# polli-labs/linnaeus

Measured on AMD Instinct MI355X. Metric: images/sec (train fwd+bwd) mFormerV1_sm 3x224x224, higher is better.
Workload: dtype bf16; 1 GPU; mFormerV1_sm train step (forward + 4-task CE loss + backward + AdamW (one HIP launch)), bf16 operands / fp32 accumulate+residual, batch 256/GPU, 3x224x224 synthetic, DropPath 0.2, gradient checkpointing off; per_gpu_batch=256, global_batch=256, parallelism=dp1, grad_mode=direct

## Files before the change

linnaeus_amd/csrc/convmlp.hip:

```cpp
#include <stdlib.h>

#include "common.hpp"
#include "../../include/lnx.h"

namespace {

struct CmP {
    const unsigned char* ln;
    const unsigned char* w1;
    const unsigned char* w2;
    const unsigned char* w2t;
    const unsigned char* w1t;
    const unsigned char* zin;
    const float* b1;
    const float* b2;
    const float* gamma;
    const float* rowscale;
    const float* x;
    const float* g;
    float* out;
    unsigned char* z;
    unsigned char* act;
    unsigned char* dh;
    unsigned char* dz;
    unsigned char* dln;
    float* dgamma;
    int M, C, rps;
    const unsigned char* y;
    const float* lnw;
    const float* lnb;
    float eps;
    unsigned char* ln_out;
    float* mean;
    float* rstd;
    float* part;
    int64_t part_floats;
    int ln_defer;
    int tile_slot;
    int dz_plain;
    float* dlnw;
    float* dlnb;
};

__device__ __forceinline__ void mfma16(f32x4_t& acc, const uint4& a, const uint4& b) {
    acc = __builtin_amdgcn_mfma_f32_16x16x32_bf16(__builtin_bit_cast(bf16x8_t, a), __builtin_bit_cast(bf16x8_t, b), acc, 0, 0, 0);
}

__device__ __forceinline__ int key4(int a) { return (4 - (a & 3)) & 3; }

#define CM_DS_READ128(dst, addr, OFF) asm volatile("ds_read_b128 %0, %1 offset:" #OFF : "=v"(dst) : "v"(addr) : "memory")

template <int NK> struct Geo {
    static constexpr int C = 32 * NK;
    static constexpr int PART = NK * 4096;
    static constexpr int CT = C / 16;
};

template <int NK, int NW>
__device__ __forceinline__ void dma_nmajor(unsigned char* lds_part, const unsigned char* W, int n0, int wave, int lane) {
    constexpr int C = Geo<NK>::C;
    constexpr int NINS = 4 * NK;
    static_assert(NINS % NW == 0, "DMA pieces must divide evenly over the waves");
#pragma unroll
    for (int t = 0; t < NINS / NW; ++t) {
        const int i = wave + NW * t;
        const int ks = i >> 2, rb = i & 3;
        const int row = 16 * rb + (lane >> 2), u = lane & 3;
        const unsigned char* src = W + ((int64_t)(n0 + row) * C + ks * 32 + ((u ^ key4(row >> 3)) << 3)) * 2;
        __builtin_amdgcn_global_load_lds((const __attribute__((address_space(1))) void*)src,
                                         (__attribute__((address_space(3))) void*)(lds_part + i * 1024), 16, 0, 0);
    }
}

template <int NK, int NW>
__device__ __forceinline__ void dma_cmajor(unsigned char* lds_part, const unsigned char* W, int n0, int wave, int lane) {
    constexpr int C = Geo<NK>::C;
    constexpr int RB = C / 16;
    constexpr int NINS = 2 * RB;
#pragma unroll
    for (int t = 0; t < NINS / NW; ++t) {
        const int i = wave + NW * t;
        const int ks2 = i / RB, rb = i % RB;
        const int row = 16 * rb + (lane >> 2), u = lane & 3;
// ... 72 lines not shown
#pragma unroll
    for (int ks2 = 0; ks2 < 2; ++ks2) {
#pragma unroll
        for (int c0 = 0; c0 < CT; c0 += GB) {
            uint4 wf[GB];
#pragma unroll
            for (int b = 0; b < GB; ++b) {
                const uint32_t a = base + (uint32_t)(ks2 * C * 64 + (c0 + b) * 1024);
                CM_DS_READ128(wf[b], a, 0);
            }
            asm volatile("s_waitcnt lgkmcnt(0)" ::: "memory");
            __builtin_amdgcn_sched_barrier(0);
#pragma unroll
            for (int b = 0; b < GB; ++b)
#pragma unroll
                for (int mt = 0; mt < MT; ++mt) mfma16(o[c0 + b][mt], wf[b], pf[mt][ks2]);
        }
    }
}

template <int NK, int MT>
__device__ __forceinline__ void prod_nmajor_pipe(f32x4_t (&h)[4][MT], uint32_t part_addr, int s, int g, const uint4 (&xf)[MT][NK]) {
    const uint32_t unit = (uint32_t)((g ^ key4(s >> 2)) << 4);
    const uint32_t base = part_addr + (uint32_t)((8 * (s >> 2) + (s & 3)) * 64) + unit;
#pragma unroll
    for (int nt = 0; nt < 4; ++nt)
#pragma unroll
        for (int mt = 0; mt < MT; ++mt) h[nt][mt] = f32x4_t{0.f, 0.f, 0.f, 0.f};
    uint4 wf[2][4];
    CM_DS_READ128(wf[0][0], base, 0);
    CM_DS_READ128(wf[0][1], base, 256);
    CM_DS_READ128(wf[0][2], base, 2048);
    CM_DS_READ128(wf[0][3], base, 2304);
#pragma unroll
    for (int ks = 0; ks < NK; ++ks) {
        if (ks + 1 < NK) {
            const uint32_t a = base + (ks + 1) * 4096;
            CM_DS_READ128(wf[(ks + 1) & 1][0], a, 0);
            CM_DS_READ128(wf[(ks + 1) & 1][1], a, 256);
            CM_DS_READ128(wf[(ks + 1) & 1][2], a, 2048);
            CM_DS_READ128(wf[(ks + 1) & 1][3], a, 2304);
            asm volatile("s_waitcnt lgkmcnt(4)" ::: "memory");
        } else {
            asm volatile("s_waitcnt lgkmcnt(0)" ::: "memory");
        }
        __builtin_amdgcn_sched_barrier(0);
#pragma unroll
        for (int nt = 0; nt < 4; ++nt)
#pragma unroll
            for (int mt = 0; mt < MT; ++mt) mfma16(h[nt][mt], wf[ks & 1][nt], xf[mt][ks]);
    }
}

template <int NK, int MT>
__device__ __forceinline__ void prod_cmajor_pipe(f32x4_t (&o)[Geo<NK>::CT][MT], uint32_t part_addr, int s, int g, const uint4 (&pf)[MT][2]) {
    constexpr int C = Geo<NK>::C;
    constexpr int CT = Geo<NK>::CT;
    const uint32_t base = part_addr + (uint32_t)(s * 64) + (uint32_t)((g ^ key4(s >> 2)) << 4);
    constexpr int GB = 4;
    constexpr int NB = 2 * CT / GB;
    static_assert(CT % GB == 0, "channel tiles must split into batches of 4");
    uint4 wf[2][GB];
#pragma unroll
    for (int b = 0; b < GB; ++b) CM_DS_READ128(wf[0][b], base + (uint32_t)(b * 1024), 0);
#pragma unroll
    for (int bt = 0; bt < NB; ++bt) {
        const int ks2 = (bt * GB) / CT, c0 = (bt * GB) % CT;
        if (bt + 1 < NB) {
            const int ks2n = ((bt + 1) * GB) / CT, c0n = ((bt + 1) * GB) % CT;
#pragma unroll
            for (int b = 0; b < GB; ++b) CM_DS_READ128(wf[(bt + 1) & 1][b], base + (uint32_t)(ks2n * C * 64 + (c0n + b) * 1024), 0);
            asm volatile("s_waitcnt lgkmcnt(4)" ::: "memory");
        } else {
            asm volatile("s_waitcnt lgkmcnt(0)" ::: "memory");
        }
        __builtin_amdgcn_sched_barrier(0);
#pragma unroll
        for (int b = 0; b < GB; ++b)
#pragma unroll
            for (int mt = 0; mt < MT; ++mt) mfma16(o[c0 + b][mt], wf[bt & 1][b], pf[mt][ks2]);
    }
}

__device__ __forceinline__ uint4 pack8(const f32x4_t& lo, const f32x4_t& hi) {
    Vec16<bf16_t> v;
#pragma unroll
    for (int j = 0; j < 4; ++j) {
        v.set(j, lo[j]);
        v.set(4 + j, hi[j]);
    }
    return v.raw;
}

__device__ __forceinline__ float g_sum(float v) {
    v += __shfl_xor(v, 16, 64);
    v += __shfl_xor(v, 32, 64);
    return v;
}
template <int CTRL> __device__ __forceinline__ float dpp_get(float v) {
    return __builtin_bit_cast(float, __builtin_amdgcn_update_dpp(0, __builtin_bit_cast(int, v), CTRL, 0xf, 0xf, false));
}
__device__ __forceinline__ float row16_sum(float v) {
    v += dpp_get<0xB1>(v);
    v += dpp_get<0x4E>(v);
    v += dpp_get<0x141>(v);
    v += dpp_get<0x140>(v);
    return v;
}
template <int NK>
__device__ __forceinline__ void ln_row_frags(uint4 (&xf)[NK], const float* w, const float* b, int g, float eps, float& mu, float& rs) {
    constexpr float invC = 1.0f / (float)Geo<NK>::C;
    float v[NK][8];
    float sum = 0.f;
#pragma unroll
    for (int ks = 0; ks < NK; ++ks) {
        Vec16<bf16_t> t;
        t.raw = xf[ks];
#pragma unroll
        for (int j = 0; j < 8; ++j) v[ks][j] = t.get(j);
        sum += ((v[ks][0] + v[ks][1]) + (v[ks][2] + v[ks][3])) + ((v[ks][4] + v[ks][5]) + (v[ks][6] + v[ks][7]));
    }
    mu = g_sum(sum) * invC;
    float sq = 0.f;
#pragma unroll
    for (int ks = 0; ks < NK; ++ks)
#pragma unroll
        for (int j = 0; j < 8; ++j) {
            v[ks][j] -= mu;
            sq = fmaf(v[ks][j], v[ks][j], sq);
        }
    rs = 1.0f / sqrtf(fmaf(g_sum(sq), invC, eps));
#pragma unroll
    for (int ks = 0; ks < NK; ++ks) {
        const int c = ks * 32 + 8 * g;
        const float4 w0 = *reinterpret_cast<const float4*>(w + c), w1 = *reinterpret_cast<const float4*>(w + c + 4);
        const float4 b0 = *reinterpret_cast<const float4*>(b + c), b1 = *reinterpret_cast<const float4*>(b + c + 4);
        const float wv[8] = {w0.x, w0.y, w0.z, w0.w, w1.x, w1.y, w1.z, w1.w};
        const float bv[8] = {b0.x, b0.y, b0.z, b0.w, b1.x, b1.y, b1.z, b1.w};
        Vec16<bf16_t> o;
#pragma unroll
        for (int j = 0; j < 8; ++j) o.set(j, fmaf(v[ks][j] * rs, wv[j], bv[j]));
        xf[ks] = o.raw;
    }
}
template <int NK>
struct LnRow {
    uint2 yr[Geo<NK>::CT];
    float mu, rs;
};
template <int NK>
__device__ __forceinline__ void ln_bwd_fetch(LnRow<NK>& r, const CmP& p, int m, int g) {
    constexpr int C = Geo<NK>::C;
    const int mc = m < p.M ? m : p.M - 1;
#pragma unroll
    for (int ct = 0; ct < Geo<NK>::CT; ++ct) r.yr[ct] = *reinterpret_cast<const uint2*>(p.y + ((int64_t)mc * C + ct * 16 + 4 * g) * 2);
    r.mu = p.mean[mc];
    r.rs = p.rstd[mc];
}
template <int NK, int MT, int MTI>
__device__ __forceinline__ void ln_bwd_rows(const CmP& p, const f32x4_t (&dl)[Geo<NK>::CT][MT], const LnRow<NK>& row, int m, int s, int g, const float* lnws,
                                            float* dls) {
    constexpr int C = Geo<NK>::C;
    constexpr int CT = Geo<NK>::CT;
    constexpr float invC = 1.0f / (float)C;
    const bool mv = m < p.M;
    const int mc = mv ? m : p.M - 1;
    const uint2 (&yr)[CT] = row.yr;
    const float mu = row.mu, rs = row.rs;
    float xh[CT][4], gv[CT][4];
    float s1 = 0.f, s2 = 0.f;
#pragma unroll
    for (int ct = 0; ct < CT; ++ct) {
        const int c = ct * 16 + 4 * g;
        const float4 w4 = *reinterpret_cast<const float4*>(lnws + c);
        const float wv[4] = {w4.x, w4.y, w4.z, w4.w};
        const bf16_t* yh = reinterpret_cast<const bf16_t*>(&yr[ct]);
#pragma unroll
        for (int r = 0; r < 4; ++r) {
            const float d = (float)(bf16_t)dl[ct][MTI][r];
            const float x = ((float)yh[r] - mu) * rs;
            xh[ct][r] = x;
            gv[ct][r] = d * wv[r];
            s1 += gv[ct][r];
            s2 = fmaf(gv[ct][r], x, s2);
            const float dm = mv ? d : 0.f;
            const float a = row16_sum(dm * x), b = row16_sum(dm);
            if (s == 0) {
                atomicAdd(&dls[c + r], a);
                atomicAdd(&dls[C + c + r], b);
            }
        }
    }
    const float m1 = g_sum(s1) * invC, m2 = g_sum(s2) * invC;
#pragma unroll
    for (int ct = 0; ct < CT; ++ct) {
        uint2 v;
        bf16_t* vh = reinterpret_cast<bf16_t*>(&v);
#pragma unroll
        for (int r = 0; r < 4; ++r) vh[r] = (bf16_t)(rs * (gv[ct][r] - m1 - xh[ct][r] * m2));
        *reinterpret_cast<uint2*>(p.dln + ((int64_t)mc * C + ct * 16 + 4 * g) * 2) = v;
    }
}

#ifdef CM_STAMP
__device__ unsigned long long g_cm_stamp[8];
#define CM_T(i) do { __builtin_amdgcn_sched_barrier(0); unsigned long long t_; asm volatile("s_memtime %0\n\ts_waitcnt lgkmcnt(0)" : "=s"(t_) :: "memory"); \
                     __builtin_amdgcn_sched_barrier(0); tsum[i] += t_ - tlast; tlast = t_; } while (0)
#else
#define CM_T(i) do { } while (0)
#endif

template <int NK, int MT, int NW, bool LNF>
__global__ __launch_bounds__(64 * NW) void convmlp_fwd_kernel(const CmP p) {
#ifdef CM_STAMP
    unsigned long long tsum[8] = {0, 0, 0, 0, 0, 0, 0, 0}, tlast;
    asm volatile("s_memtime %0\n\ts_waitcnt lgkmcnt(0)" : "=s"(tlast)::"memory");
#endif
    constexpr int C = Geo<NK>::C;
    constexpr int CT = Geo<NK>::CT;
    constexpr int PART = Geo<NK>::PART;
    constexpr int STAGE = 2 * PART;
    constexpr int NCH = 4 * C / 64;
    constexpr int NLD = 8 * NK / NW;
    extern __shared__ __attribute__((aligned(16))) unsigned char smem[];
    float* b1s = reinterpret_cast<float*>(smem + 3 * STAGE);

    const int lane = threadIdx.x & 63;
    const int wave = __builtin_amdgcn_readfirstlane(threadIdx.x >> 6);
    const int s = lane & 15, g = lane >> 4;
    const int m_base = blockIdx.x * (16 * NW * MT) + wave * (16 * MT);
    const uint32_t lds0 = (uint32_t)(uintptr_t)(__attribute__((address_space(3))) unsigned char*)smem;

    for (int i = threadIdx.x; i < 4 * C; i += 64 * NW) b1s[i] = p.b1[i];

    uint4 xf[MT][NK];
#pragma unroll
    for (int mt = 0; mt < MT; ++mt) {
        int m = m_base + mt * 16 + s;
        if (m >= p.M) m = p.M - 1;
#pragma unroll
        for (int ks = 0; ks < NK; ++ks) xf[mt][ks] = ld16((LNF ? p.y : p.ln) + ((int64_t)m * C + ks * 32 + 8 * g) * 2);
    }
    if constexpr (LNF) {
#pragma unroll
        for (int mt = 0; mt < MT; ++mt) {
            float mu, rs;
            ln_row_frags<NK>(xf[mt], p.lnw, p.lnb, g, p.eps, mu, rs);
            const int m = m_base + mt * 16 + s;
            if (m < p.M) {
                if (p.ln_out) {
#pragma unroll
                    for (int ks = 0; ks < NK; ++ks) st16(p.ln_out + ((int64_t)m * C + ks * 32 + 8 * g) * 2, xf[mt][ks]);
                }
                if (p.mean && g == 0) {
                    p.mean[m] = mu;
                    p.rstd[m] = rs;
                }
            }
        }
    }
    f32x4_t o[CT][MT];
#pragma unroll
    for (int ct = 0; ct < CT; ++ct)
#pragma unroll
        for (int mt = 0; mt < MT; ++mt) o[ct][mt] = f32x4_t{0.f, 0.f, 0.f, 0.f};

    __syncthreads();
    dma_nmajor<NK, NW>(smem, p.w1, 0, wave, lane);
    dma_cmajor<NK, NW>(smem + PART, p.w2, 0, wave, lane);
    dma_nmajor<NK, NW>(smem + STAGE, p.w1, 64, wave, lane);
    dma_cmajor<NK, NW>(smem + STAGE + PART, p.w2, 64, wave, lane);
    CM_T(0);
    for (int j = 0; j < NCH; ++j) {
        const int stg = j % 3;
        if (j + 1 < NCH) asm volatile("s_waitcnt vmcnt(%0)" ::"n"(NLD) : "memory");
        else asm volatile("s_waitcnt vmcnt(0)" ::: "memory");
        CM_T(1);
        __builtin_amdgcn_s_barrier();
        CM_T(2);
        if (j + 2 < NCH) {
            unsigned char* nx = smem + ((j + 2) % 3) * STAGE;
            dma_nmajor<NK, NW>(nx, p.w1, 64 * (j + 2), wave, lane);
            dma_cmajor<NK, NW>(nx + PART, p.w2, 64 * (j + 2), wave, lane);
        }
        const uint32_t st = lds0 + stg * STAGE;
        f32x4_t h[4][MT];
        CM_T(3);
        prod_nmajor_pipe<NK, MT>(h, st, s, g, xf);
        CM_T(4);
        uint4 pf[MT][2];
        {
            f32x4_t bv[4];
            const uint32_t ba = lds0 + 3 * STAGE + (uint32_t)((64 * j + 8 * g) * 4);
            CM_DS_READ128(bv[0], ba, 0);
            CM_DS_READ128(bv[1], ba, 16);
            CM_DS_READ128(bv[2], ba, 128);
            CM_DS_READ128(bv[3], ba, 144);
            asm volatile("s_waitcnt lgkmcnt(0)" ::: "memory");
            __builtin_amdgcn_sched_barrier(0);
#pragma unroll
            for (int mt = 0; mt < MT; ++mt)
#pragma unroll
                for (int n2 = 0; n2 < 4; n2 += 2) {
                    f32x4_t hv[2] = {h[n2][mt], h[n2 + 1][mt]};
                    gelu4_bias_n<2>(hv, &bv[n2]);
                    h[n2][mt] = hv[0];
                    h[n2 + 1][mt] = hv[1];
                }
#pragma unroll
            for (int mt = 0; mt < MT; ++mt) {
                pf[mt][0] = pack8(h[0][mt], h[1][mt]);
                pf[mt][1] = pack8(h[2][mt], h[3][mt]);
            }
        }
        CM_T(5);
        prod_cmajor_pipe<NK, MT>(o, st + PART, s, g, pf);
        CM_T(6);
    }
#pragma unroll
    for (int mt = 0; mt < MT; ++mt) {
        const int m = m_base + mt * 16 + s;
        if (m >= p.M) continue;
        const float rs = p.rowscale ? p.rowscale[m / p.rps] : 1.0f;
        float4 xrv[CT], b2v[CT], gmv[CT];
#pragma unroll
        for (int ct = 0; ct < CT; ++ct) {
            const int c = ct * 16 + 4 * g;
            xrv[ct] = *reinterpret_cast<const float4*>(p.x + (int64_t)m * C + c);
            b2v[ct] = *reinterpret_cast<const float4*>(p.b2 + c);
            gmv[ct] = *reinterpret_cast<const float4*>(p.gamma + c);
        }
#pragma unroll
        for (int ct = 0; ct < CT; ++ct) {
            const int c = ct * 16 + 4 * g;
            const float4 b2 = b2v[ct], gm = gmv[ct], xr = xrv[ct];
            const float z0 = o[ct][mt][0] + b2.x, z1 = o[ct][mt][1] + b2.y, z2 = o[ct][mt][2] + b2.z, z3 = o[ct][mt][3] + b2.w;
            if (p.z) {
                uint2 zz;
                bf16_t* zh = reinterpret_cast<bf16_t*>(&zz);
                zh[0] = (bf16_t)z0; zh[1] = (bf16_t)z1; zh[2] = (bf16_t)z2; zh[3] = (bf16_t)z3;
                *reinterpret_cast<uint2*>(p.z + ((int64_t)m * C + c) * 2) = zz;
            }
            *reinterpret_cast<float4*>(p.out + (int64_t)m * C + c) =
                make_float4(xr.x + rs * gm.x * z0, xr.y + rs * gm.y * z1, xr.z + rs * gm.z * z2, xr.w + rs * gm.w * z3);
        }
    }
    CM_T(7);
#ifdef CM_STAMP
    if (blockIdx.x == gridDim.x / 2 && threadIdx.x == 0)
        for (int i = 0; i < 8; ++i) g_cm_stamp[i] = tsum[i];
#endif
}
#ifdef CM_STAMP
extern "C" int lnx_dbg_convmlp_stamps(unsigned long long* out8) { return (int)hipMemcpyFromSymbol(out8, HIP_SYMBOL(g_cm_stamp), 64); }
#endif

template <int NK, int MT, int NW, bool ST, bool LNB, bool DG>
__global__ __launch_bounds__(64 * NW) void convmlp_bwd_kernel(const CmP p) {
    constexpr int C = Geo<NK>::C;
    constexpr int CT = Geo<NK>::CT;
    constexpr int PART = Geo<NK>::PART;
    constexpr int STAGE = 3 * PART;
    constexpr int NCH = 4 * C / 64;
    constexpr int NLD = 12 * NK / NW;
    extern __shared__ __attribute__((aligned(16))) unsigned char smem[];
    float* b1s = reinterpret_cast<float*>(smem + 2 * STAGE);
    float* dgs = b1s + 4 * C;
    float* lws = dgs + C;
    float* dls = lws + C;

    const int lane = threadIdx.x & 63;
    const int wave = __builtin_amdgcn_readfirstlane(threadIdx.x >> 6);
    const int s = lane & 15, g = lane >> 4;
    const int m_base = blockIdx.x * (16 * NW * MT) + wave * (16 * MT);
    const uint32_t lds0 = (uint32_t)(uintptr_t)(__attribute__((address_space(3))) unsigned char*)smem;

    for (int i = threadIdx.x; i < 4 * C; i += 64 * NW) b1s[i] = p.b1[i];
    for (int i = threadIdx.x; i < C; i += 64 * NW) {
        dgs[i] = 0.f;
        if constexpr (LNB) {
            lws[i] = p.lnw[i];
            dls[i] = dls[C + i] = 0.f;
        }
    }
    __syncthreads();

    uint4 xf[MT][NK], zf[MT][NK];
    bool mvalid[MT];
#pragma unroll
    for (int mt = 0; mt < MT; ++mt) {
        int m = m_base + mt * 16 + s;
        mvalid[mt] = m < p.M;
        if (!mvalid[mt]) m = p.M - 1;
        const float rs = p.rowscale ? p.rowscale[m / p.rps] : 1.0f;
        float4 g0v[NK], g1v[NK], a0v[NK], a1v[NK];
        uint4 zraw[NK];
#pragma unroll
        for (int ks = 0; ks < NK; ++ks) {
            const int c = ks * 32 + 8 * g;
            xf[mt][ks] = ld16(p.ln + ((int64_t)m * C + c) * 2);
            g0v[ks] = *reinterpret_cast<const float4*>(p.g + (int64_t)m * C + c);
            g1v[ks] = *reinterpret_cast<const float4*>(p.g + (int64_t)m * C + c + 4);
            a0v[ks] = *reinterpret_cast<const float4*>(p.gamma + c);
            a1v[ks] = *reinterpret_cast<const float4*>(p.gamma + c + 4);
            if constexpr (DG) zraw[ks] = ld16(p.zin + ((int64_t)m * C + c) * 2);
        }
#pragma unroll
        for (int ks = 0; ks < NK; ++ks) {
            const int c = ks * 32 + 8 * g;
            const float4 g0 = g0v[ks], g1 = g1v[ks], a0 = a0v[ks], a1 = a1v[ks];
            Vec16<bf16_t> zin, dzv, dzs;
            if constexpr (DG) zin.raw = zraw[ks];
            const float gv[8] = {g0.x, g0.y, g0.z, g0.w, g1.x, g1.y, g1.z, g1.w};
            const float av[8] = {a0.x, a0.y, a0.z, a0.w, a1.x, a1.y, a1.z, a1.w};
#pragma unroll
            for (int j = 0; j < 8; ++j) {
                const float sg = rs * gv[j];
                dzv.set(j, sg * av[j]);
                dzs.set(j, p.dz_plain ? sg : sg * av[j]);
                if constexpr (DG) {
                    const float dgp = mvalid[mt] ? sg * zin.get(j) : 0.f;
                    float t = dgp;
                    t += __shfl_xor(t, 1, 64);
                    t += __shfl_xor(t, 2, 64);
                    t += __shfl_xor(t, 4, 64);
                    t += __shfl_xor(t, 8, 64);
                    if (s == 0) atomicAdd(&dgs[c + j], t);
                }
            }
            zf[mt][ks] = dzv.raw;
            st16(p.dz + ((int64_t)m * C + c) * 2, dzs.raw);
        }
    }
    f32x4_t dl[CT][MT];
#pragma unroll
    for (int ct = 0; ct < CT; ++ct)
#pragma unroll
        for (int mt = 0; mt < MT; ++mt) dl[ct][mt] = f32x4_t{0.f, 0.f, 0.f, 0.f};
    LnRow<NK> lrow;
    if constexpr (LNB) ln_bwd_fetch<NK>(lrow, p, m_base + s, g);

    __syncthreads();
    dma_nmajor<NK, NW>(smem, p.w1, 0, wave, lane);
    dma_nmajor<NK, NW>(smem + PART, p.w2t, 0, wave, lane);
    dma_cmajor<NK, NW>(smem + 2 * PART, p.w1t, 0, wave, lane);
    for (int j = 0; j < NCH; ++j) {
        const int stg = j & 1;
        __builtin_amdgcn_s_barrier();
        if (j + 1 < NCH) {
            unsigned char* nx = smem + (stg ^ 1) * STAGE;
            dma_nmajor<NK, NW>(nx, p.w1, 64 * (j + 1), wave, lane);
            dma_nmajor<NK, NW>(nx + PART, p.w2t, 64 * (j + 1), wave, lane);
            dma_cmajor<NK, NW>(nx + 2 * PART, p.w1t, 64 * (j + 1), wave, lane);
            asm volatile("s_waitcnt vmcnt(%0)" ::"n"(NLD) : "memory");
        } else {
            asm volatile("s_waitcnt vmcnt(0)" ::: "memory");
        }
        __builtin_amdgcn_s_barrier();
        const uint32_t st = lds0 + stg * STAGE;
        f32x4_t h[4][MT], da[4][MT];
        prod_nmajor_pipe<NK, MT>(h, st, s, g, xf);
        prod_nmajor_pipe<NK, MT>(da, st + PART, s, g, zf);
        f32x4_t bv[4];
        const uint32_t ba = lds0 + 2 * STAGE + (uint32_t)((64 * j + 8 * g) * 4);
        CM_DS_READ128(bv[0], ba, 0);
        CM_DS_READ128(bv[1], ba, 16);
        CM_DS_READ128(bv[2], ba, 128);
        CM_DS_READ128(bv[3], ba, 144);
        asm volatile("s_waitcnt lgkmcnt(0)" ::: "memory");
        __builtin_amdgcn_sched_barrier(0);
#pragma unroll
        for (int mt = 0; mt < MT; ++mt)
#pragma unroll
            for (int n2 = 0; n2 < 4; n2 += 2) {
                f32x4_t hv[2] = {h[n2][mt], h[n2 + 1][mt]}, dv[2] = {da[n2][mt], da[n2 + 1][mt]};
                gelu4_bias_grad_n<2>(hv, &bv[n2], dv);
                h[n2][mt] = hv[0];
                h[n2 + 1][mt] = hv[1];
                da[n2][mt] = dv[0];
                da[n2 + 1][mt] = dv[1];
            }
        uint4 pa[MT][2], pd[MT][2];
#pragma unroll
        for (int mt = 0; mt < MT; ++mt) {
            pa[mt][0] = pack8(h[0][mt], h[1][mt]);
            pa[mt][1] = pack8(h[2][mt], h[3][mt]);
            pd[mt][0] = pack8(da[0][mt], da[1][mt]);
            pd[mt][1] = pack8(da[2][mt], da[3][mt]);
            const int m = min(m_base + mt * 16 + s, p.M - 1);
            if constexpr (ST) {
                const int64_t off = ((int64_t)m * (4 * C) + 64 * j + 8 * g) * 2;
                st16(p.act + off, pa[mt][0]);
                st16(p.act + off + 64, pa[mt][1]);
                st16(p.dh + off, pd[mt][0]);
                st16(p.dh + off + 64, pd[mt][1]);
            }
        }
        prod_cmajor_pipe<NK, MT>(dl, st + 2 * PART, s, g, pd);
    }
    if constexpr (LNB) {
        static_assert(MT == 1, "ln_bwd_rows is instantiated per m-tile");
        ln_bwd_rows<NK, MT, 0>(p, dl, lrow, m_base + s, s, g, lws, dls);
    } else {
#pragma unroll
        for (int mt = 0; mt < MT; ++mt) {
            const int m = min(m_base + mt * 16 + s, p.M - 1);
#pragma unroll
            for (int ct = 0; ct < CT; ++ct) {
                const int c = ct * 16 + 4 * g;
                uint2 v;
                bf16_t* vh = reinterpret_cast<bf16_t*>(&v);
                vh[0] = (bf16_t)dl[ct][mt][0]; vh[1] = (bf16_t)dl[ct][mt][1]; vh[2] = (bf16_t)dl[ct][mt][2]; vh[3] = (bf16_t)dl[ct][mt][3];
                *reinterpret_cast<uint2*>(p.dln + ((int64_t)m * C + c) * 2) = v;
            }
        }
    }
    __syncthreads();
    if constexpr (DG)
        for (int i = threadIdx.x; i < C; i += 64 * NW) atomicAdd(p.dgamma + i, dgs[i]);
    if constexpr (LNB)
        for (int i = threadIdx.x; i < 2 * C; i += 64 * NW) p.part[(int64_t)blockIdx.x * (2 * C) + i] = dls[i];
}


template <int NK>
__device__ __forceinline__ void dma_all_nmajor(unsigned char* img, const unsigned char* W, int wave, int lane) {
    constexpr int C = Geo<NK>::C;
    constexpr int NCH = 4 * C / 64;
    constexpr int NINS = 4 * NK;
    for (int q = wave; q < NCH * NINS; q += 8) {
        const int j = q / NINS, i = q % NINS;
        const int ks = i >> 2, rb = i & 3;
        const int row = 16 * rb + (lane >> 2), u = lane & 3;
        const unsigned char* src = W + ((int64_t)(64 * j + row) * C + ks * 32 + ((u ^ key4(row >> 3)) << 3)) * 2;
        __builtin_amdgcn_global_load_lds((const __attribute__((address_space(1))) void*)src,
                                         (__attribute__((address_space(3))) void*)(img + j * Geo<NK>::PART + i * 1024), 16, 0, 0);
    }
}
template <int NK>
__device__ __forceinline__ void dma_all_cmajor(unsigned char* img, const unsigned char* W, int wave, int lane) {
    constexpr int C = Geo<NK>::C;
    constexpr int NCH = 4 * C / 64;
    constexpr int RB = C / 16;
    constexpr int NINS = 2 * RB;
    for (int q = wave; q < NCH * NINS; q += 8) {
        const int j = q / NINS, i = q % NINS;
        const int ks2 = i / RB, rb = i % RB;
        const int row = 16 * rb + (lane >> 2), u = lane & 3;
        const unsigned char* src = W + ((int64_t)row * (4 * C) + 64 * j + ks2 * 32 + ((u ^ key4(row >> 2)) << 3)) * 2;
        __builtin_amdgcn_global_load_lds((const __attribute__((address_space(1))) void*)src,
                                         (__attribute__((address_space(3))) void*)(img + j * Geo<NK>::PART + i * 1024), 16, 0, 0);
    }
}

typedef __attribute__((ext_vector_type(4))) short cm_s16x4;
template <int NK, int MT>
__device__ __forceinline__ void prod_tr_nmajor(f32x4_t (&o)[Geo<NK>::CT][MT], uint32_t part_addr, int s, int g, const uint4 (&pf)[MT][2]) {
    constexpr int CT = Geo<NK>::CT;
    const int q = s >> 2, pp = s & 3;
#pragma unroll
    for (int ks2 = 0; ks2 < 2; ++ks2) {
        const int n = 32 * ks2 + 8 * g + q;
        uint2 lo[CT], hi[CT];
#pragma unroll
        for (int ct = 0; ct < CT; ++ct) {
            const int ks = ct >> 1;
            const int unit = 2 * (ct & 1) + (pp >> 1);
            const uint32_t a = part_addr + (uint32_t)(ks * 4096 + n * 64 + ((unit ^ key4(g)) << 4) + (pp & 1) * 8);
            asm volatile("ds_read_b64_tr_b16 %0, %1" : "=v"(lo[ct]) : "v"(a) : "memory");
            asm volatile("ds_read_b64_tr_b16 %0, %1 offset:256" : "=v"(hi[ct]) : "v"(a) : "memory");
        }
        asm volatile("s_waitcnt lgkmcnt(0)" ::: "memory");
        __builtin_amdgcn_sched_barrier(0);
#pragma unroll
        for (int ct = 0; ct < CT; ++ct) {
            const uint4 wf = make_uint4(lo[ct].x, lo[ct].y, hi[ct].x, hi[ct].y);
#pragma unroll
            for (int mt = 0; mt < MT; ++mt) mfma16(o[ct][mt], wf, pf[mt][ks2]);
        }
    }
}

template <bool V> struct BoolC { static constexpr bool value = V; };
template <int NK, bool LNF, int SAVE>
__global__ __launch_bounds__(512) void convmlp_fwd_res_kernel(const CmP p) {
    constexpr int MT = 2;
    constexpr int C = Geo<NK>::C;
    constexpr int CT = Geo<NK>::CT;
    constexpr int PART = Geo<NK>::PART;
    constexpr int NCH = 4 * C / 64;
    extern __shared__ __attribute__((aligned(16))) unsigned char smem[];
    unsigned char* w1img = smem;
    unsigned char* w2img = smem + NCH * PART;
    float* b1s = reinterpret_cast<float*>(smem + 2 * NCH * PART);
    float* b2s = b1s + 4 * C;
    float* gms = b2s + C;
    float* lws = gms + C;
    float* lbs = lws + C;
    const int lane = threadIdx.x & 63;
    const int wave = __builtin_amdgcn_readfirstlane(threadIdx.x >> 6);
    const int s = lane & 15, g = lane >> 4;
    const uint32_t lds0 = (uint32_t)(uintptr_t)(__attribute__((address_space(3))) unsigned char*)smem;

    for (int i = threadIdx.x; i < 4 * C; i += 512) b1s[i] = p.b1[i];
    for (int i = threadIdx.x; i < C; i += 512) {
        b2s[i] = p.b2[i];
        gms[i] = p.gamma[i];
        if constexpr (LNF) {
            lws[i] = p.lnw[i];
            lbs[i] = p.lnb[i];
        }
    }
    const bool dyn = p.tile_slot >= 0;
    const TileShare sh = tile_share((p.M + 31) / 32);
    unsigned* const ctr = &g_tile_ctr[dyn ? p.tile_slot : 0][sh.part][0];
    int drawn = dyn ? sched_draw_counted(ctr) : 0;
    dma_all_nmajor<NK>(w1img, p.w1, wave, lane);
    dma_all_cmajor<NK>(w2img, p.w2, wave, lane);
    asm volatile("s_waitcnt vmcnt(0)" ::: "memory");
    __syncthreads();

    const int ntile = (p.M + 31) / 32;
    auto load_x = [&](uint4 (&dst)[MT][NK], int tile) __attribute__((always_inline)) {
#pragma unroll
        for (int mt = 0; mt < MT; ++mt) {
            const int m = min(tile * 32 + mt * 16 + s, p.M - 1);
#pragma unroll
            for (int ks = 0; ks < NK; ++ks) dst[mt][ks] = ld16((LNF ? p.y : p.ln) + ((int64_t)m * C + ks * 32 + 8 * g) * 2);
        }
    };
    const int xbase = sh.base, xcnt = sh.cnt, xwaves = 8 * sh.workers;
    const int last_draw = xcnt + xwaves - 1;
    int pos = dyn ? __builtin_amdgcn_readfirstlane(drawn) : sh.index * 8 + wave;
    bool reset_ctr = dyn && pos == last_draw;
    uint4 xf[MT][NK];
    if (pos < xcnt) load_x(xf, xbase + pos);
    const float* rsp = p.rowscale ? p.rowscale : p.gamma;
    const float rsf = p.rowscale ? 1.0f : 0.0f;

    int next = 0;
    for (; pos < xcnt; pos = next) {
        const int tile = xbase + pos;
        const int m_base = tile * 32;
        if constexpr (LNF) {
#pragma unroll
            for (int mt = 0; mt < MT; ++mt) {
                float mu, rs;
                ln_row_frags<NK>(xf[mt], lws, lbs, g, p.eps, mu, rs);
                const int m = min(m_base + mt * 16 + s, p.M - 1);
                if constexpr (SAVE != 0) {
#pragma unroll
                    for (int ks = 0; ks < NK; ++ks) st16(p.ln_out + ((int64_t)m * C + ks * 32 + 8 * g) * 2, xf[mt][ks]);
                    if (g == 0) {
                        p.mean[m] = mu;
                        p.rstd[m] = rs;
                    }
                }
            }
        }
        if constexpr (LNF) __builtin_amdgcn_sched_barrier(0);
        if (dyn) drawn = sched_draw_counted(ctr);
        float4 xrv[MT][CT];
// ... 312 lines not shown
        return grid > 256 ? 256 : grid;
    }
    return cdiv(M, 16 * (nw8 ? 8 : 4));
}

static int res_room() {
    const int cus = device_cus();
    const int room = persistent_cus(cus > 0 ? cus : 256);
    return room > 256 ? 256 : room;
}

template <int NK, bool LNF, int SAVE>
int launch_fwd_res_t(const CmP& p, hipStream_t st) {
    const size_t lds = 2 * (4 * Geo<NK>::C / 64) * Geo<NK>::PART + 8 * Geo<NK>::C * sizeof(float);
    static bool attr = false;
    if (!attr) {
        (void)hipFuncSetAttribute(reinterpret_cast<const void*>(&convmlp_fwd_res_kernel<NK, LNF, SAVE>), hipFuncAttributeMaxDynamicSharedMemorySize, (int)lds);
        attr = true;
    }
    int grid = cdiv(cdiv(p.M, 32), 8);
    const int room = res_room();
    if (grid > room) grid = room;
    CmP q = p;
    q.tile_slot = tile_sched_static() ? -1 : tile_slot_of(st);
    hipLaunchKernelGGL((convmlp_fwd_res_kernel<NK, LNF, SAVE>), dim3(grid), dim3(512), lds, st, q);
    return 0;
}
template <int NK>
int launch_fwd_res(const CmP& p, hipStream_t st) {
    if (p.y) return p.z ? launch_fwd_res_t<NK, true, 1>(p, st) : (p.ln_out ? launch_fwd_res_t<NK, true, 2>(p, st) : launch_fwd_res_t<NK, true, 0>(p, st));
    return p.z ? launch_fwd_res_t<NK, false, 1>(p, st) : launch_fwd_res_t<NK, false, 0>(p, st);
}
inline int reduce_ln_partials(const CmP& p, int nwg, hipStream_t st) {
    if (p.ln_defer) {
        ln_postpone_reduce(p.part, nwg, p.C, p.dlnw, p.dlnb, nwg >= 64 ? 64 : 1, st);
        return 0;
    }
    hipLaunchKernelGGL(ln_partials_reduce_kernel, dim3(cdiv(2 * p.C, 256), nwg >= 64 ? 64 : 1), dim3(256), 0, st, p.part, nwg, p.C, p.dlnw, p.dlnb);
    return 0;
}
template <int NK, int MT, bool ST, bool LNB, bool DG>
int launch_bwd_res_t(const CmP& p, hipStream_t st) {
    const size_t lds = 2 * (4 * Geo<NK>::C / 64) * Geo<NK>::PART + 9 * Geo<NK>::C * sizeof(float);
    static bool attr = false;
    if (!attr) {
        (void)hipFuncSetAttribute(reinterpret_cast<const void*>(&convmlp_bwd_res_kernel<NK, MT, ST, LNB, DG>), hipFuncAttributeMaxDynamicSharedMemorySize, (int)lds);
        attr = true;
    }
    int grid = bwd_grid(p.C, p.M);
    if (LNB && (int64_t)grid * 2 * p.C > p.part_floats) return -1;
    const int room = res_room();
    if (grid > room) grid = room;
    CmP q = p;
    q.tile_slot = tile_sched_static() ? -1 : tile_slot_of(st);
    hipLaunchKernelGGL((convmlp_bwd_res_kernel<NK, MT, ST, LNB, DG>), dim3(grid), dim3(512), lds, st, q);
    return LNB ? reduce_ln_partials(p, grid, st) : 0;
}
template <int NK, int MT>
int launch_bwd_res(const CmP& p, hipStream_t st) {
    if (p.zin == nullptr) {
        if (p.y) return p.act ? launch_bwd_res_t<NK, MT, true, true, false>(p, st) : launch_bwd_res_t<NK, MT, false, true, false>(p, st);
        return p.act ? launch_bwd_res_t<NK, MT, true, false, false>(p, st) : launch_bwd_res_t<NK, MT, false, false, false>(p, st);
    }
    if (p.y) return p.act ? launch_bwd_res_t<NK, MT, true, true, true>(p, st) : launch_bwd_res_t<NK, MT, false, true, true>(p, st);
    return p.act ? launch_bwd_res_t<NK, MT, true, false, true>(p, st) : launch_bwd_res_t<NK, MT, false, false, true>(p, st);
}

template <int NK, int MT, int NW, bool LNF>
int launch_fwd_t(const CmP& p, hipStream_t st) {
    const size_t lds = 3 * 2 * Geo<NK>::PART + 4 * Geo<NK>::C * sizeof(float);
    static bool attr = false;
    if (!attr) {
        (void)hipFuncSetAttribute(reinterpret_cast<const void*>(&convmlp_fwd_kernel<NK, MT, NW, LNF>), hipFuncAttributeMaxDynamicSharedMemorySize, (int)lds);
        attr = true;
    }
    hipLaunchKernelGGL((convmlp_fwd_kernel<NK, MT, NW, LNF>), dim3(cdiv(p.M, 16 * NW * MT)), dim3(64 * NW), lds, st, p);
    return 0;
}
template <int NK, int MT, int NW>
int launch_fwd(const CmP& p, hipStream_t st) {
    return p.y ? launch_fwd_t<NK, MT, NW, true>(p, st) : launch_fwd_t<NK, MT, NW, false>(p, st);
}

template <int NK, int MT, int NW, bool ST, bool LNB, bool DG>
int launch_bwd_t(const CmP& p, hipStream_t st) {
    const size_t lds = 2 * 3 * Geo<NK>::PART + 8 * Geo<NK>::C * sizeof(float);
    static bool attr = false;
    if (!attr) {
        (void)hipFuncSetAttribute(reinterpret_cast<const void*>(&convmlp_bwd_kernel<NK, MT, NW, ST, LNB, DG>), hipFuncAttributeMaxDynamicSharedMemorySize, (int)lds);
        attr = true;
    }
    static_assert(MT == 1, "bwd_grid() assumes 16-row wave tiles in the streamed-weight backward");
    const int grid = bwd_grid(p.C, p.M);
    if (LNB && (int64_t)grid * 2 * p.C > p.part_floats) return -1;
    hipLaunchKernelGGL((convmlp_bwd_kernel<NK, MT, NW, ST, LNB, DG>), dim3(grid), dim3(64 * NW), lds, st, p);
    return LNB ? reduce_ln_partials(p, grid, st) : 0;
}
template <int NK, int MT, int NW>
int launch_bwd(const CmP& p, hipStream_t st) {
    if (p.zin == nullptr) {
        if (p.y) return p.act ? launch_bwd_t<NK, MT, NW, true, true, false>(p, st) : launch_bwd_t<NK, MT, NW, false, true, false>(p, st);
        return p.act ? launch_bwd_t<NK, MT, NW, true, false, false>(p, st) : launch_bwd_t<NK, MT, NW, false, false, false>(p, st);
    }
    if (p.y) return p.act ? launch_bwd_t<NK, MT, NW, true, true, true>(p, st) : launch_bwd_t<NK, MT, NW, false, true, true>(p, st);
    return p.act ? launch_bwd_t<NK, MT, NW, true, false, true>(p, st) : launch_bwd_t<NK, MT, NW, false, false, true>(p, st);
}

}

extern "C" int64_t lnx_convmlp_bwd_ws_floats(int C, int M) {
    if (!lnx_convmlp_supported(LNX_BF16, C) || M <= 0) return 0;
    return (int64_t)bwd_grid(C, M) * 2 * C;
}

extern "C" int lnx_convmlp_supported(int dtype, int C) { return dtype == LNX_BF16 && (C == 32 || C == 64 || C == 96 || C == 128 || C == 192); }

extern "C" int lnx_convmlp_fwd(const lnx_convmlp_args* a, void* stream) {
    LNX_CHECK(a && (a->ln || a->y) && a->w1 && a->w2 && a->b1 && a->b2 && a->gamma && a->x && a->out, "lnx_convmlp_fwd: null operand");
    if (a->y) {
        LNX_CHECK(a->ln_w && a->ln_b && a->ln == nullptr, "lnx_convmlp_fwd: the fused LayerNorm form takes y, ln_w, ln_b and no ln");
        LNX_CHECK((a->mean == nullptr) == (a->ln_out == nullptr) && (a->rstd == nullptr) == (a->ln_out == nullptr) && (a->z == nullptr || a->ln_out != nullptr),
                  "lnx_convmlp_fwd: with y, the outputs ln_out, mean and rstd are written together (what a backward needs) or not at all; z only with them");
    }
    LNX_CHECK(lnx_convmlp_supported(a->dtype, a->C), "lnx_convmlp_fwd: unsupported dtype %d / C %d (bf16, C in {32,64,96,128,192})", a->dtype, a->C);
    LNX_CHECK(a->M > 0, "lnx_convmlp_fwd: empty");
    if (a->rowscale) LNX_CHECK(a->rows_per_sample > 0, "lnx_convmlp_fwd: rowscale needs rows_per_sample");
    CmP p{};
    p.ln = (const unsigned char*)a->ln; p.w1 = (const unsigned char*)a->w1; p.w2 = (const unsigned char*)a->w2;
    p.b1 = a->b1; p.b2 = a->b2; p.gamma = a->gamma; p.rowscale = a->rowscale; p.x = a->x; p.out = a->out; p.z = (unsigned char*)a->z;
    p.M = a->M; p.C = a->C; p.rps = a->rows_per_sample > 0 ? a->rows_per_sample : 1;
    p.y = (const unsigned char*)a->y; p.lnw = a->ln_w; p.lnb = a->ln_b; p.eps = a->ln_eps; p.ln_out = (unsigned char*)a->ln_out; p.mean = a->mean; p.rstd = a->rstd;
    hipStream_t st = (hipStream_t)stream;
    switch (a->C) {
        case 32: launch_fwd_res<1>(p, st); break;
        case 64: launch_fwd_res<2>(p, st); break;
        case 96: launch_fwd_res<3>(p, st); break;
        case 128: if (nw8) launch_fwd<4, 1, 8>(p, st); else launch_fwd<4, 1, 4>(p, st); break;
        case 192: if (nw8) launch_fwd<6, 1, 8>(p, st); else launch_fwd<6, 1, 4>(p, st); break;
    }
    LNX_LAUNCH_CHECK();
    return 0;
}

extern "C" int lnx_convmlp_bwd(const lnx_convmlp_bwd_args* a, void* stream) {
    LNX_CHECK(a && a->g && a->ln && a->w1 && a->w2t && a->w1t && a->b1 && a->gamma && a->dz && a->dln && (a->dgamma || !a->z),
              "lnx_convmlp_bwd: null operand (z may be NULL: dgamma is then not produced here; with z, dgamma is required)");
    LNX_CHECK((a->act == nullptr) == (a->dh == nullptr), "lnx_convmlp_bwd: act and dh must both be given or both be NULL");
    LNX_CHECK(lnx_convmlp_supported(a->dtype, a->C), "lnx_convmlp_bwd: unsupported dtype %d / C %d", a->dtype, a->C);
    LNX_CHECK(a->M > 0, "lnx_convmlp_bwd: empty");
    if (a->rowscale) LNX_CHECK(a->rows_per_sample > 0, "lnx_convmlp_bwd: rowscale needs rows_per_sample");
    if (a->y) LNX_CHECK(a->ln_w && a->mean && a->rstd && a->d_ln_w && a->d_ln_b && a->ws, "lnx_convmlp_bwd: the fused LayerNorm form needs ln_w, mean, rstd, d_ln_w, d_ln_b and ws");
    CmP p{};
    p.y = (const unsigned char*)a->y; p.lnw = a->ln_w; p.mean = const_cast<float*>(a->mean); p.rstd = const_cast<float*>(a->rstd);
    p.part = a->ws; p.part_floats = a->ws_floats; p.dlnw = a->d_ln_w; p.dlnb = a->d_ln_b; p.ln_defer = a->ln_defer;
    p.g = a->g; p.ln = (const unsigned char*)a->ln; p.zin = (const unsigned char*)a->z; p.w1 = (const unsigned char*)a->w1;
    p.w2t = (const unsigned char*)a->w2t; p.w1t = (const unsigned char*)a->w1t; p.b1 = a->b1; p.gamma = a->gamma; p.rowscale = a->rowscale;
    p.act = (unsigned char*)a->act; p.dh = (unsigned char*)a->dh; p.dz = (unsigned char*)a->dz; p.dln = (unsigned char*)a->dln; p.dgamma = a->dgamma;
    p.M = a->M; p.C = a->C; p.rps = a->rows_per_sample > 0 ? a->rows_per_sample : 1;
    p.dz_plain = a->dz_plain != 0;
    hipStream_t st = (hipStream_t)stream;
    int rc = 0;
    switch (a->C) {
        case 32: rc = launch_bwd_res<1, 2>(p, st); break;
        case 64: rc = launch_bwd_res<2, 1>(p, st); break;
        case 96: rc = launch_bwd_res<3, 1>(p, st); break;
        case 128: rc = nw8 ? launch_bwd<4, 1, 8>(p, st) : launch_bwd<4, 1, 4>(p, st); break;
        case 192: rc = nw8 ? launch_bwd<6, 1, 8>(p, st) : launch_bwd<6, 1, 4>(p, st); break;
    }
    LNX_CHECK(rc == 0, "lnx_convmlp_bwd: ws too small for the LayerNorm partial sums (M=%d C=%d ws_floats=%lld)", a->M, a->C, (long long)a->ws_floats);
    LNX_LAUNCH_CHECK();
    return 0;
}
```

Baseline: 13310 images/sec.

## Drop w1t stream in ConvMLP backward via transposed LDS reads, triple-buffer weights

The streamed-weight ConvMLP backward (C=128/192) now defaults to reading W1 transposed directly from LDS with ds_read_b64_tr_b16 instead of streaming a separate pre-transposed w1t copy. The freed LDS lets each stage hold only w1 and w2t, so the loop uses three stages with prefetch two chunks ahead and a single barrier per chunk. Weight DMA for the first two chunks is issued before the activation loads to overlap them. This cuts global weight traffic and barrier count at the cost of transposed-read LDS latency; the old form stays behind an env var, and timing stamps are added under a debug macro.

After: 13430 images/sec, median of 6. Within noise of the previous version (+0.9%).

```diff
diff --git a/linnaeus_amd/csrc/convmlp.hip b/linnaeus_amd/csrc/convmlp.hip
--- a/linnaeus_amd/csrc/convmlp.hip
+++ b/linnaeus_amd/csrc/convmlp.hip
@@ -1,4 +1,5 @@
 #include <stdlib.h>
+#include <string.h>
 
 #include "common.hpp"
 #include "../../include/lnx.h"
@@ -237,6 +238,34 @@
     }
 }
 
+typedef __attribute__((ext_vector_type(4))) short cm_s16x4;
+template <int NK, int MT>
+__device__ __forceinline__ void prod_tr_nmajor(f32x4_t (&o)[Geo<NK>::CT][MT], uint32_t part_addr, int s, int g, const uint4 (&pf)[MT][2]) {
+    constexpr int CT = Geo<NK>::CT;
+    const int q = s >> 2, pp = s & 3;
+#pragma unroll
+    for (int ks2 = 0; ks2 < 2; ++ks2) {
+        const int n = 32 * ks2 + 8 * g + q;
+        uint2 lo[CT], hi[CT];
+#pragma unroll
+        for (int ct = 0; ct < CT; ++ct) {
+            const int ks = ct >> 1;
+            const int unit = 2 * (ct & 1) + (pp >> 1);
+            const uint32_t a = part_addr + (uint32_t)(ks * 4096 + n * 64 + ((unit ^ key4(g)) << 4) + (pp & 1) * 8);
+            asm volatile("ds_read_b64_tr_b16 %0, %1" : "=v"(lo[ct]) : "v"(a) : "memory");
+            asm volatile("ds_read_b64_tr_b16 %0, %1 offset:256" : "=v"(hi[ct]) : "v"(a) : "memory");
+        }
+        asm volatile("s_waitcnt lgkmcnt(0)" ::: "memory");
+        __builtin_amdgcn_sched_barrier(0);
+#pragma unroll
+        for (int ct = 0; ct < CT; ++ct) {
+            const uint4 wf = make_uint4(lo[ct].x, lo[ct].y, hi[ct].x, hi[ct].y);
+#pragma unroll
+            for (int mt = 0; mt < MT; ++mt) mfma16(o[ct][mt], wf, pf[mt][ks2]);
+        }
+    }
+}
+
 __device__ __forceinline__ uint4 pack8(const f32x4_t& lo, const f32x4_t& hi) {
     Vec16<bf16_t> v;
 #pragma unroll
@@ -359,6 +388,7 @@
 
 #ifdef CM_STAMP
 __device__ unsigned long long g_cm_stamp[8];
+__device__ unsigned long long g_cmb_stamp[10];
 #define CM_T(i) do { __builtin_amdgcn_sched_barrier(0); unsigned long long t_; asm volatile("s_memtime %0\n\ts_waitcnt lgkmcnt(0)" : "=s"(t_) :: "memory"); \
                      __builtin_amdgcn_sched_barrier(0); tsum[i] += t_ - tlast; tlast = t_; } while (0)
 #else
@@ -508,18 +538,26 @@
 }
 #ifdef CM_STAMP
 extern "C" int lnx_dbg_convmlp_stamps(unsigned long long* out8) { return (int)hipMemcpyFromSymbol(out8, HIP_SYMBOL(g_cm_stamp), 64); }
+extern "C" int lnx_dbg_convmlp_bwd_stamps(unsigned long long* out10) { return (int)hipMemcpyFromSymbol(out10, HIP_SYMBOL(g_cmb_stamp), 80); }
 #endif
 
-template <int NK, int MT, int NW, bool ST, bool LNB, bool DG>
+template <int NK, int MT, int NW, bool ST, bool LNB, bool DG, bool W1T>
 __global__ __launch_bounds__(64 * NW) void convmlp_bwd_kernel(const CmP p) {
+#ifdef CM_STAMP
+    unsigned long long tsum[10] = {0, 0, 0, 0, 0, 0, 0, 0, 0, 0}, tlast;
+    asm volatile("s_memtime %0\n\ts_waitcnt lgkmcnt(0)" : "=s"(tlast)::"memory");
+#endif
     constexpr int C = Geo<NK>::C;
     constexpr int CT = Geo<NK>::CT;
     constexpr int PART = Geo<NK>::PART;
-    constexpr int STAGE = 3 * PART;
+    constexpr int NPART = W1T ? 3 : 2;
+    constexpr int NSTG = W1T ? 2 : 3;
+    constexpr int STAGE = NPART * PART;
     constexpr int NCH = 4 * C / 64;
-    constexpr int NLD = 12 * NK / NW;
+    constexpr int NLD = 4 * NPART * NK / NW;
+    constexpr int NST = ST ? 4 * MT : 0;
     extern __shared__ __attribute__((aligned(16))) unsigned char smem[];
-    float* b1s = reinterpret_cast<float*>(smem + 2 * STAGE);
+    float* b1s = reinterpret_cast<float*>(smem + NSTG * STAGE);
     float* dgs = b1s + 4 * C;
     float* lws = dgs + C;
     float* dls = lws + C;
@@ -539,6 +577,18 @@
         }
     }
     __syncthreads();
+    auto issue = [&](int j) __attribute__((always_inline)) {
+        unsigned char* nx = smem + (j % NSTG) * STAGE;
+        dma_nmajor<NK, NW>(nx, p.w1, 64 * j, wave, lane);
+        dma_nmajor<NK, NW>(nx + PART, p.w2t, 64 * j, wave, lane);
+        if constexpr (W1T) dma_cmajor<NK, NW>(nx + 2 * PART, p.w1t, 64 * j, wave, lane);
+    };
+    if constexpr (!W1T) {
+        issue(0);
+        issue(1);
+    }
+    LnRow<NK> lrow;
+    if constexpr (LNB && !W1T) ln_bwd_fetch<NK>(lrow, p, m_base + s, g);
 
     uint4 xf[MT][NK], zf[MT][NK];
     bool mvalid[MT];
@@ -592,32 +642,45 @@
     for (int ct = 0; ct < CT; ++ct)
 #pragma unroll
         for (int mt = 0; mt < MT; ++mt) dl[ct][mt] = f32x4_t{0.f, 0.f, 0.f, 0.f};
-    LnRow<NK> lrow;
-    if constexpr (LNB) ln_bwd_fetch<NK>(lrow, p, m_base + s, g);
-
-    __syncthreads();
-    dma_nmajor<NK, NW>(smem, p.w1, 0, wave, lane);
-    dma_nmajor<NK, NW>(smem + PART, p.w2t, 0, wave, lane);
-    dma_cmajor<NK, NW>(smem + 2 * PART, p.w1t, 0, wave, lane);
+    if constexpr (W1T) {
+        if constexpr (LNB) ln_bwd_fetch<NK>(lrow, p, m_base + s, g);
+        __syncthreads();
+        issue(0);
+    }
+    CM_T(0);
+#pragma unroll 1
     for (int j = 0; j < NCH; ++j) {
-        const int stg = j & 1;
-        __builtin_amdgcn_s_barrier();
-        if (j + 1 < NCH) {
-            unsigned char* nx = smem + (stg ^ 1) * STAGE;
-            dma_nmajor<NK, NW>(nx, p.w1, 64 * (j + 1), wave, lane);
-            dma_nmajor<NK, NW>(nx + PART, p.w2t, 64 * (j + 1), wave, lane);
-            dma_cmajor<NK, NW>(nx + 2 * PART, p.w1t, 64 * (j + 1), wave, lane);
-            asm volatile("s_waitcnt vmcnt(%0)" ::"n"(NLD) : "memory");
+        if constexpr (W1T) {
+            __builtin_amdgcn_s_barrier();
+            CM_T(2);
+            if (j + 1 < NCH) {
+                issue(j + 1);
+                CM_T(3);
+                asm volatile("s_waitcnt vmcnt(%0)" ::"n"(NLD) : "memory");
+            } else {
+                asm volatile("s_waitcnt vmcnt(0)" ::: "memory");
+            }
+            CM_T(1);
+            __builtin_amdgcn_s_barrier();
+            CM_T(2);
         } else {
-            asm volatile("s_waitcnt vmcnt(0)" ::: "memory");
-        }
-        __builtin_amdgcn_s_barrier();
-        const uint32_t st = lds0 + stg * STAGE;
+            if (j == 0) asm volatile("s_waitcnt vmcnt(%0)" ::"n"(NLD) : "memory");
+            else if (j + 1 < NCH) asm volatile("s_waitcnt vmcnt(%0)" ::"n"(NLD + NST) : "memory");
+            else asm volatile("s_waitcnt vmcnt(0)" ::: "memory");
+            CM_T(1);
+            __builtin_amdgcn_s_barrier();
+            CM_T(2);
+            if (j + 2 < NCH) issue(j + 2);
+            CM_T(3);
+        }
+        const uint32_t st = lds0 + (j % NSTG) * STAGE;
         f32x4_t h[4][MT], da[4][MT];
         prod_nmajor_pipe<NK, MT>(h, st, s, g, xf);
+        CM_T(4);
         prod_nmajor_pipe<NK, MT>(da, st + PART, s, g, zf);
+        CM_T(5);
         f32x4_t bv[4];
-        const uint32_t ba = lds0 + 2 * STAGE + (uint32_t)((64 * j + 8 * g) * 4);
+        const uint32_t ba = lds0 + NSTG * STAGE + (uint32_t)((64 * j + 8 * g) * 4);
         CM_DS_READ128(bv[0], ba, 0);
         CM_DS_READ128(bv[1], ba, 16);
         CM_DS_READ128(bv[2], ba, 128);
@@ -635,6 +698,7 @@
                 da[n2][mt] = dv[0];
                 da[n2 + 1][mt] = dv[1];
             }
+        CM_T(6);
         uint4 pa[MT][2], pd[MT][2];
 #pragma unroll
         for (int mt = 0; mt < MT; ++mt) {
@@ -651,7 +715,10 @@
                 st16(p.dh + off + 64, pd[mt][1]);
             }
         }
-        prod_cmajor_pipe<NK, MT>(dl, st + 2 * PART, s, g, pd);
+        CM_T(7);
+        if constexpr (W1T) prod_cmajor_pipe<NK, MT>(dl, st + 2 * PART, s, g, pd);
+        else prod_tr_nmajor<NK, MT>(dl, st, s, g, pd);
+        CM_T(8);
     }
     if constexpr (LNB) {
         static_assert(MT == 1, "ln_bwd_rows is instantiated per m-tile");
@@ -675,6 +742,11 @@
         for (int i = threadIdx.x; i < C; i += 64 * NW) atomicAdd(p.dgamma + i, dgs[i]);
     if constexpr (LNB)
         for (int i = threadIdx.x; i < 2 * C; i += 64 * NW) p.part[(int64_t)blockIdx.x * (2 * C) + i] = dls[i];
+    CM_T(9);
+#ifdef CM_STAMP
+    if (blockIdx.x == gridDim.x / 2 && threadIdx.x == 0)
+        for (int i = 0; i < 10; ++i) g_cmb_stamp[i] = tsum[i];
+#endif
 }
 
 
@@ -705,34 +777,6 @@
         const unsigned char* src = W + ((int64_t)row * (4 * C) + 64 * j + ks2 * 32 + ((u ^ key4(row >> 2)) << 3)) * 2;
         __builtin_amdgcn_global_load_lds((const __attribute__((address_space(1))) void*)src,
                                          (__attribute__((address_space(3))) void*)(img + j * Geo<NK>::PART + i * 1024), 16, 0, 0);
-    }
-}
-
-typedef __attribute__((ext_vector_type(4))) short cm_s16x4;
-template <int NK, int MT>
-__device__ __forceinline__ void prod_tr_nmajor(f32x4_t (&o)[Geo<NK>::CT][MT], uint32_t part_addr, int s, int g, const uint4 (&pf)[MT][2]) {
-    constexpr int CT = Geo<NK>::CT;
-    const int q = s >> 2, pp = s & 3;
-#pragma unroll
-    for (int ks2 = 0; ks2 < 2; ++ks2) {
-        const int n = 32 * ks2 + 8 * g + q;
-        uint2 lo[CT], hi[CT];
-#pragma unroll
-        for (int ct = 0; ct < CT; ++ct) {
-            const int ks = ct >> 1;
-            const int unit = 2 * (ct & 1) + (pp >> 1);
-            const uint32_t a = part_addr + (uint32_t)(ks * 4096 + n * 64 + ((unit ^ key4(g)) << 4) + (pp & 1) * 8);
-            asm volatile("ds_read_b64_tr_b16 %0, %1" : "=v"(lo[ct]) : "v"(a) : "memory");
-            asm volatile("ds_read_b64_tr_b16 %0, %1 offset:256" : "=v"(hi[ct]) : "v"(a) : "memory");
-        }
-        asm volatile("s_waitcnt lgkmcnt(0)" ::: "memory");
-        __builtin_amdgcn_sched_barrier(0);
-#pragma unroll
-        for (int ct = 0; ct < CT; ++ct) {
-            const uint4 wf = make_uint4(lo[ct].x, lo[ct].y, hi[ct].x, hi[ct].y);
-#pragma unroll
-            for (int mt = 0; mt < MT; ++mt) mfma16(o[ct][mt], wf, pf[mt][ks2]);
-        }
     }
 }
 
@@ -1211,28 +1255,38 @@
     return p.y ? launch_fwd_t<NK, MT, NW, true>(p, st) : launch_fwd_t<NK, MT, NW, false>(p, st);
 }
 
-template <int NK, int MT, int NW, bool ST, bool LNB, bool DG>
+static bool bwd_w1t_form() {
+    const char* e = getenv("LNX_CM_BWD");
+    return e && strcmp(e, "w1t") == 0;
+}
+
+template <int NK, int MT, int NW, bool ST, bool LNB, bool DG, bool W1T>
 int launch_bwd_t(const CmP& p, hipStream_t st) {
     const size_t lds = 2 * 3 * Geo<NK>::PART + 8 * Geo<NK>::C * sizeof(float);
     static bool attr = false;
     if (!attr) {
-        (void)hipFuncSetAttribute(reinterpret_cast<const void*>(&convmlp_bwd_kernel<NK, MT, NW, ST, LNB, DG>), hipFuncAttributeMaxDynamicSharedMemorySize, (int)lds);
+        (void)hipFuncSetAttribute(reinterpret_cast<const void*>(&convmlp_bwd_kernel<NK, MT, NW, ST, LNB, DG, W1T>), hipFuncAttributeMaxDynamicSharedMemorySize, (int)lds);
         attr = true;
     }
     static_assert(MT == 1, "bwd_grid() assumes 16-row wave tiles in the streamed-weight backward");
     const int grid = bwd_grid(p.C, p.M);
     if (LNB && (int64_t)grid * 2 * p.C > p.part_floats) return -1;
-    hipLaunchKernelGGL((convmlp_bwd_kernel<NK, MT, NW, ST, LNB, DG>), dim3(grid), dim3(64 * NW), lds, st, p);
+    hipLaunchKernelGGL((convmlp_bwd_kernel<NK, MT, NW, ST, LNB, DG, W1T>), dim3(grid), dim3(64 * NW), lds, st, p);
     return LNB ? reduce_ln_partials(p, grid, st) : 0;
 }
-template <int NK, int MT, int NW>
+template <int NK, int MT, int NW, bool W1T>
+int launch_bwd_f(const CmP& p, hipStream_t st) {
+    if (p.zin == nullptr) {
+        if (p.y) return p.act ? launch_bwd_t<NK, MT, NW, true, true, false, W1T>(p, st) : launch_bwd_t<NK, MT, NW, false, true, false, W1T>(p, st);
+        return p.act ? launch_bwd_t<NK, MT, NW, true, false, false, W1T>(p, st) : launch_bwd_t<NK, MT, NW, false, false, false, W1T>(p, st);
+    }
+    if (p.y) return p.act ? launch_bwd_t<NK, MT, NW, true, true, true, W1T>(p, st) : launch_bwd_t<NK, MT, NW, false, true, true, W1T>(p, st);
+    return p.act ? launch_bwd_t<NK, MT, NW, true, false, true, W1T>(p, st) : launch_bwd_t<NK, MT, NW, false, false, true, W1T>(p, st);
+}
+template <int NK, int MT>
 int launch_bwd(const CmP& p, hipStream_t st) {
-    if (p.zin == nullptr) {
-        if (p.y) return p.act ? launch_bwd_t<NK, MT, NW, true, true, false>(p, st) : launch_bwd_t<NK, MT, NW, false, true, false>(p, st);
-        return p.act ? launch_bwd_t<NK, MT, NW, true, false, false>(p, st) : launch_bwd_t<NK, MT, NW, false, false, false>(p, st);
-    }
-    if (p.y) return p.act ? launch_bwd_t<NK, MT, NW, true, true, true>(p, st) : launch_bwd_t<NK, MT, NW, false, true, true>(p, st);
-    return p.act ? launch_bwd_t<NK, MT, NW, true, false, true>(p, st) : launch_bwd_t<NK, MT, NW, false, false, true>(p, st);
+    if (!nw8) return launch_bwd_f<NK, MT, 4, false>(p, st);
+    return bwd_w1t_form() ? launch_bwd_f<NK, MT, 8, true>(p, st) : launch_bwd_f<NK, MT, 8, false>(p, st);
 }
 
 }
@@ -1293,8 +1347,8 @@
         case 32: rc = launch_bwd_res<1, 2>(p, st); break;
         case 64: rc = launch_bwd_res<2, 1>(p, st); break;
         case 96: rc = launch_bwd_res<3, 1>(p, st); break;
-        case 128: rc = nw8 ? launch_bwd<4, 1, 8>(p, st) : launch_bwd<4, 1, 4>(p, st); break;
-        case 192: rc = nw8 ? launch_bwd<6, 1, 8>(p, st) : launch_bwd<6, 1, 4>(p, st); break;
+        case 128: rc = launch_bwd<4, 1>(p, st); break;
+        case 192: rc = launch_bwd<6, 1>(p, st); break;
     }
     LNX_CHECK(rc == 0, "lnx_convmlp_bwd: ws too small for the LayerNorm partial sums (M=%d C=%d ws_floats=%lld)", a->M, a->C, (long long)a->ws_floats);
     LNX_LAUNCH_CHECK();
```
